# APRIL-ZJU/Ctrl-VIO

Measured on AMD Instinct MI355X. Metric: sliding-window solves/sec (10 KF, 200 lm, 2000 IMU), higher is better.
Workload: dtype f64; 1 GPU; config2: 10 KF / 200 landmarks / 2000 IMU sliding window (K = 24 knots, 814 reprojection blocks), <= 15 LM iterations (Ceres 1.14 trust region + projected line search); distinct_windows_per_gpu=64, streams_per_gpu=4, concurrent_solves_per_gpu=2

## Files before the change

ctrl-vio_amd/csrc/kernels.hpp:

```cpp
#pragma once
#include <utility>

#include "device_types.hpp"
#include "factors.hpp"

namespace ctv {

enum { LIN_AT_X = 0,
       LIN_SPEC = 1,
       COST_AT_X = 2 };
__device__ __forceinline__ bool lin_run(const Lm &lm, int mode) { return lm.status == 0 && (mode != LIN_SPEC || lm.step_valid != 0); }
__device__ __forceinline__ bool lin_cost_only(const Lm &lm, int mode, const LmParams &p) {
  return mode == COST_AT_X || (mode == LIN_SPEC && lm.iter >= p.max_iters && lm.ls_active == 0);
}
__device__ __forceinline__ int lin_target(const Lm &lm, int mode) { return mode == LIN_SPEC ? 1 - lm.cur : lm.cur; }

__device__ __forceinline__ double grad_norm_entry(const Dev &d, const WinMeta &m, int w, int j, const double *g, bool at_cand);
__device__ __forceinline__ void begin_iteration(const Dev &d, int w, int *s_go);

__device__ __forceinline__ double readlane_d(double x, int lane) {
  const long long b = __double_as_longlong(x);
  const int lo = __builtin_amdgcn_readlane((int)(b & 0xffffffffll), lane);
  const int hi = __builtin_amdgcn_readlane((int)(b >> 32), lane);
  return __longlong_as_double(((long long)hi << 32) | (unsigned int)lo);
}

__device__ __forceinline__ int opaque_zero() {
  int z;
  asm volatile("s_mov_b32 %0, 0" : "=s"(z));
  return z;
}

__device__ __forceinline__ void lds_wave_sync() {
  __builtin_amdgcn_s_waitcnt(0xc07f);
  __builtin_amdgcn_wave_barrier();
}
__device__ __forceinline__ void lds_block_sync() {
  __builtin_amdgcn_s_waitcnt(0xc07f);
  __builtin_amdgcn_s_barrier();
}

#define CTV_STAMP(stamps, idx, cap, lane_cond, ...)                                                        \
  do {                                                                                                     \
    if ((stamps) && (lane_cond) && (idx) < (cap))                                                          \
      (stamps)[(idx)++] = clock64() __VA_OPT__(+ (long long)((__VA_ARGS__) * 0.0));                        \
  } while (0)

__device__ __forceinline__ int imu_col(int c, int s, int K, int bias) {
  if (c < 12) return 6 * (s + c / 3) + c % 3;
  if (c < 24) return 6 * (s + (c - 12) / 3) + 3 + (c - 12) % 3;
  return 6 * K + 6 * bias + (c - 24);
}
__device__ __forceinline__ int vis_col(int c, int si, int sj, int P) {
  if (c < 12) return 6 * (si + c / 3) + c % 3;
  if (c < 24) return 6 * (si + (c - 12) / 3) + 3 + (c - 12) % 3;
  if (c < 36) return 6 * (sj + (c - 24) / 3) + (c - 24) % 3;
  if (c < 48) return 6 * (sj + (c - 36) / 3) + 3 + (c - 36) % 3;
  if (c == 48) return -1;
  return P - 1;
}

__device__ __forceinline__ void load_knots(const double *quat, const double *pos, int k0, const double *origin,
                                                            Knots4 &k) {
#pragma unroll
  for (int i = 0; i < 4; ++i) {
    const double *q = quat + 4 * (k0 + i), *p = pos + 3 * (k0 + i);
    k.q[i] = qmk(q[0], q[1], q[2], q[3]);
    k.p[i] = mk(p[0] - origin[0], p[1] - origin[1], p[2] - origin[2]);
  }
}

struct LocalFrame {
  Q4 qref_inv;
  M3 RT;
  double o[3];
  __device__ __forceinline__ void init(const double *quat, const double *pos, int kref) {
    const double *q = quat + 4 * kref, *p = pos + 3 * kref;
    qref_inv = qmk(-q[0], -q[1], -q[2], q[3]);
    const M3 R = q2R(qmk(q[0], q[1], q[2], q[3]));
#pragma unroll
    for (int i = 0; i < 3; ++i)
#pragma unroll
      for (int j = 0; j < 3; ++j) RT.m[3 * i + j] = R.m[3 * j + i];
    o[0] = p[0]; o[1] = p[1]; o[2] = p[2];
  }
  __device__ __forceinline__ void load(const double *quat, const double *pos, int k0, Knots4 &k) const {
#pragma unroll
    for (int i = 0; i < 4; ++i) {
      const double *q = quat + 4 * (k0 + i), *p = pos + 3 * (k0 + i);
      k.q[i] = qmul_raw(qref_inv, qmk(q[0], q[1], q[2], q[3]));
      k.p[i] = mul(RT, mk(p[0] - o[0], p[1] - o[1], p[2] - o[2]));
    }
  }
  __device__ __forceinline__ V3 rotate(const double *v) const { return mul(RT, mk(v[0], v[1], v[2])); }
  __device__ __forceinline__ M3 RrefT() const { return RT; }
};

}

#include "kernels_control.hpp"
#include "kernels_imu.hpp"
#include "kernels_visual.hpp"
#include "kernels_assemble.hpp"
#include "kernels_solve.hpp"
#include "kernels_query.hpp"
#include "kernels_cov.hpp"
#include "kernels_tri.hpp"
```

ctrl-vio_amd/csrc/kernels_assemble.hpp:

```cpp
#pragma once

namespace ctv {

__device__ __forceinline__ double prior_H(const Dev &d, const WinMeta &m, int ga, int gb) {
  if (m.pn <= 0) return 0.0;
  const int pi = d.pinv[m.p0 + ga], pj = d.pinv[m.p0 + gb];
  return (pi >= 0 && pj >= 0) ? d.pH[m.pH0 + (size_t)pi * m.pn + pj] : 0.0;
}
__device__ __forceinline__ double prior_g(const Dev &d, const WinMeta &m, int u) {
  if (m.pn <= 0) return 0.0;
  const int pi = d.pinv[m.p0 + u];
  return pi >= 0 ? d.pgrad[m.pv0 + pi] : 0.0;
}
__device__ __forceinline__ void packed_decode(int i, int tri, int K6, int P, int &ga, int &gb) {
  if (i < tri) {
    ga = (int)((sqrtf(8.0f * (float)i + 1.0f) - 1.0f) * 0.5f);
    ga += ((ga + 1) * (ga + 2) / 2 <= i) ? 1 : 0;
    ga -= (ga * (ga + 1) / 2 > i) ? 1 : 0;
    gb = i - ga * (ga + 1) / 2;
  } else {
    ga = P - 1;
    gb = (i - tri) < K6 ? (i - tri) : P - 1;
  }
}
__device__ __forceinline__ void bias_rows_store(const Dev &d, const WinMeta &m, int tg, const double *bias, int first, int stride) {
  const int K = m.K, F = m.F, P = m.P, K6 = 6 * K, ldh = m.ldh, nbr = 6 * F;
  double *Hg = d.HppS[tg] + m.H0, *g = d.gS[tg] + m.u0;
  const int32_t *boff = d.bgl_off + m.bias0 + (int)(&m - d.wins);
  const int n_rect = nbr * K6, n_tri = nbr * (nbr + 1) / 2, n_ld = nbr, n_g = nbr;
  for (int e = first; e < n_rect + n_tri + n_ld + n_g; e += stride) {
    if (e < n_rect + n_tri) {
      int rb, c;
      if (e < n_rect) { rb = e / K6; c = e - rb * K6; }
      else {
        const int t = e - n_rect;
        int i2 = (int)((sqrtf(8.0f * (float)t + 1.0f) - 1.0f) * 0.5f);
        i2 += ((i2 + 1) * (i2 + 2) / 2 <= t) ? 1 : 0;
        i2 -= (i2 * (i2 + 1) / 2 > t) ? 1 : 0;
        rb = i2; c = K6 + t - i2 * (i2 + 1) / 2;
      }
      const int f = rb / 6, a = rb - 6 * f, r = K6 + rb;
      double v = 0.0;
      const int g0 = boff[f], g1 = boff[f + 1];
      if (c < K6) {
        const int k = c / 6, cc = c - 6 * k;
        for (int q = g0; q < g1; ++q) {
          const int gi = d.bgl[q];
          const int sg = d.groups[gi].s;
          if (k >= sg && k <= sg + 3) v += d.imu_tiles[(size_t)gi * 1024 + (24 + a) * 32 + (cc < 3 ? 3 * (k - sg) + cc : 12 + 3 * (k - sg) + cc - 3)];
        }
      } else {
        const int cb = c - K6, f2 = cb / 6, a2 = cb - 6 * f2;
        if (f2 == f)
          for (int q = g0; q < g1; ++q) v += d.imu_tiles[(size_t)d.bgl[q] * 1024 + (24 + a) * 32 + 24 + a2];
        if (a2 == a)
          for (int b = 0; b < m.NB; ++b) {
            const int bi = d.bc_i[m.bc0 + b], bj = d.bc_j[m.bc0 + b];
            const double wv = d.bc_w[(size_t)(m.bc0 + b) * 6 + a];
            if (f2 == f) { if (bi == f) v += wv * wv; if (bj == f) v += wv * wv; }
            else if ((bi == f2 && bj == f) || (bi == f && bj == f2)) v -= wv * wv;
          }
      }
      Hg[(long long)r * ldh + c] = v + prior_H(d, m, r, c);
    } else if (e < n_rect + n_tri + n_ld) {
      const int c = K6 + e - n_rect - n_tri;
      Hg[(long long)(P - 1) * ldh + c] = prior_H(d, m, P - 1, c);
    } else {
      const int rb = e - n_rect - n_tri - n_ld, f = rb / 6, a = rb - 6 * f, r = K6 + rb;
      double v = 0.0;
      for (int q = boff[f]; q < boff[f + 1]; ++q) v += d.imu_tiles[(size_t)d.bgl[q] * 1024 + (24 + a) * 32 + 30];
      for (int b = 0; b < m.NB; ++b) {
        const int bi = d.bc_i[m.bc0 + b], bj = d.bc_j[m.bc0 + b];
        if (bi != f && bj != f) continue;
        const double wv = d.bc_w[(size_t)(m.bc0 + b) * 6 + a];
        const double rr = wv * (bias[6 * (m.bias0 + bj) + a] - bias[6 * (m.bias0 + bi) + a]);
        if (bi == f) v -= wv * rr;
        if (bj == f) v += wv * rr;
      }
      g[r] = v + prior_g(d, m, r);
    }
  }
}

constexpr int VIS_SROWS = 116;
constexpr int vis_stage_stride(int ch) { return ch + 1; }
constexpr size_t vis_stage_bytes(int nw, int ch) { return (size_t)nw * VIS_SROWS * vis_stage_stride(ch) * sizeof(double) + (size_t)nw * 2 * ch * sizeof(int); }
__device__ __forceinline__ f64x4 mfma16(double a, double b, f64x4 c) { return __builtin_amdgcn_mfma_f64_16x16x4f64(a, b, c, 0, 0, 0); }
template <int CH, bool LDSH, int NW = 8, bool STORE = false> __global__ __launch_bounds__(64 * NW) void k_assemble_vis_mfma(Dev d, int mode) {
  typedef f64x4 acc_t;
  constexpr int CHP = vis_stage_stride(CH), RPP = 64 / CH, NT = 64 * NW;
  static_assert(!STORE || LDSH, "the store-semantics tail needs the LDS-resident Hessian");
  static_assert(CH == 8, "the staging pattern is written for items of 8 blocks");
  constexpr int SROWS = VIS_SROWS, NEXP = 48 / RPP;
  const long long t_begin = d.dbg ? clock64() : 0;
  const int w = blockIdx.x, part = blockIdx.y, nparts = gridDim.y;
  if (!lin_run(d.lm[w], mode) || lin_cost_only(d.lm[w], mode, d.prm)) return;
  const WinMeta &m = d.wins[w];
  const int tgset = lin_target(d.lm[w], mode);
  const int P = m.P, K = m.K, nvitem = m.nvitem, vitem0 = m.vitem0, ngrp = m.ngrp, grp0 = m.grp0, u0 = m.u0, ldh = m.ldh;
  if ((m.vis_lds != 0) != LDSH) return;
  if (!LDSH && m.V == 0) return;
  extern __shared__ __attribute__((aligned(16))) unsigned char smv[];
  double *Hs = reinterpret_cast<double *>(smv);
  const int K6 = 6 * K, tri = K6 * (K6 + 1) / 2;
  const int nHh = LDSH ? tri + K6 + 1 : 0;
  const int nH = nHh + K6 + 1;
  double *gs = Hs + nHh;
  double *stage = reinterpret_cast<double *>(Hs + ((nH + 3) & ~3));
  int *keys = reinterpret_cast<int *>(stage + NW * SROWS * CHP);
  const int tid = threadIdx.x, wave = tid >> 6, lane = tid & 63;
  const int per_round = NW * nparts;
  constexpr int NGI = 3;
  double tv[NGI][9], tgv[NGI];
  int gs_[NGI], gb_[NGI];
  if (LDSH) {
#pragma unroll
    for (int u = 0; u < NGI; ++u) {
      const int gi = min(part * NW + wave + u * per_round, max(ngrp - 1, 0));
      const ImuGroup grp = d.groups[grp0 + gi];
      gs_[u] = grp.s; gb_[u] = grp.bias;
      const double *tile = d.imu_tiles + (size_t)(grp0 + gi) * 1024;
#pragma unroll
      for (int q = 0; q < 9; ++q) { const int e = lane + 64 * q; tv[u][q] = ngrp > 0 ? tile[(e / 24) * 32 + e % 24] : 0.0; }
      tgv[u] = (STORE && ngrp > 0) ? tile[min(lane, 23) * 32 + 30] : 0.0;
    }
  }
  for (int i = 2 * tid; i < ((nH + 3) & ~3); i += 2 * NT) *reinterpret_cast<double2 *>(Hs + i) = double2{0.0, 0.0};
  __syncthreads();
  if (LDSH) {
#pragma unroll
    for (int u = 0; u < NGI; ++u) {
      if (part * NW + wave + u * per_round >= ngrp) continue;
#pragma unroll
      for (int q = 0; q < 9; ++q) {
        const int e = lane + 64 * q, a = e / 24, b = e % 24;
        const int ga = imu_col(a, gs_[u], K, gb_[u]), gb = imu_col(b, gs_[u], K, gb_[u]);
        if (ga >= gb) atomicAdd(&Hs[ga * (ga + 1) / 2 + gb], tv[u][q]);
      }
      if (STORE && lane < 24) atomicAdd(&Hs[nHh + imu_col(lane, gs_[u], K, gb_[u])], tgv[u]);
    }
  }
  double *Js = stage + wave * SROWS * CHP;
  int *ks = keys + wave * 2 * CH;
  const size_t V = (size_t)d.Vtot;
  const int it0 = (int)((long long)nvitem * (part * NW + wave) / per_round);
  const int rounds = (int)((long long)nvitem * (part * NW + wave + 1) / per_round) - it0;
  double *Hg = d.HppS[tgset] + m.H0;
  const int q4 = lane >> 4, l15 = lane & 15, bsel = q4 >> 1, rr = q4 & 1;
  const int sc = lane % CH, srr = lane / CH;
  long long *dbg = (d.dbg && w == (d.nwin > 1000 ? 1000 : 0) && part == 0) ? d.dbg + 48 : nullptr;
  int dbi = 0;
  if (dbg && tid == 0) dbg[dbi++] = t_begin;
  CTV_STAMP(dbg, dbi, 15, tid == 0);
  int orow[3];
#pragma unroll
  for (int I = 0; I < 3; ++I) orow[I] = (2 * (16 * I + l15) + rr) * CHP;
  const int ldrow = (98 + rr) * CHP, rrow = (100 + rr) * CHP;
  double tj[5], tg9[9], tc0 = 0.0;
  int n = 0, v0 = 0, key_i = 0, key_j = 0;
  int my_start, my_count;
  {
    const int it = it0 + lane;
    const VisItem I = d.vitems[vitem0 + min(it, max(nvitem - 1, 0))];
    my_start = I.start;
    my_count = (lane < rounds && it < nvitem) ? I.count : 0;
  }
  auto item_desc = [&](int r, int &istart, int &icount) {
    if (r < 64) { istart = __shfl(my_start, r); icount = __shfl(my_count, r); }
    else {
      const int it = it0 + r;
      const VisItem I = d.vitems[vitem0 + min(it, nvitem - 1)];
      istart = I.start; icount = (r < rounds && it < nvitem) ? I.count : 0;
    }
    if (r >= rounds) icount = 0;
  };
  int idn = 0, idkn = 0, ian = 0, iakn = 0;
  auto load_ids = [&](int r) {
    int istart, icount;
    item_desc(r, istart, icount);
    idn = d.vblk[istart + (sc < icount ? sc : 0)];
    ian = d.vblk_anc[istart + (sc < icount ? sc : 0)];
    idkn = d.vblk[istart + (lane < icount ? lane : 0)];
    iakn = d.vblk_anc[istart + (lane < icount ? lane : 0)];
  };
  auto fetch = [&](int r) {
    int istart, icount;
    item_desc(r, istart, icount);
    n = icount;
    v0 = istart;
    const unsigned jb = (unsigned)idn * (unsigned)VT_ROWS + (unsigned)srr;
#pragma unroll
    for (int i = 0; i < 3; ++i) tj[i] = d.Jt[jb + (unsigned)(8 * i)];
    tj[3] = d.Jt[jb + 26u];
    tj[4] = d.Jt[(unsigned)idn * (unsigned)VT_ROWS + (unsigned)min(34 + srr, VT_ROWS - 1)];
    const double *rec = d.arec + (size_t)ian * AREC;
#pragma unroll
    for (int i = 0; i < 3; ++i)
#pragma unroll
      for (int mm = 0; mm < 3; ++mm) tg9[3 * i + mm] = rec[AR_GR + 3 * ((srr + 8 * i) >> 1) + mm];
    tc0 = rec[AR_CP0 + (srr & 3)];
    key_i = d.a_s[iakn];
    key_j = d.vsj[idkn];
    load_ids(r + 1);
  };
  if (nvitem > 0) load_ids(0);
  if (nvitem > 0) fetch(0);
  acc_t acc[6];
  double pl[3], pr[3], pll, prl;
  int asi = -1, asj = -1;
  auto reset_acc = [&]() {
#pragma unroll
    for (int q = 0; q < 6; ++q) acc[q] = acc_t{0.0, 0.0, 0.0, 0.0};
#pragma unroll
    for (int I = 0; I < 3; ++I) { pl[I] = 0.0; pr[I] = 0.0; }
    pll = 0.0; prl = 0.0;
  };
  auto scatter = [&](int si, int sj) {
#pragma unroll
    for (int I = 0; I < 3; ++I) {
      pl[I] += __shfl_xor(pl[I], 16); pl[I] += __shfl_xor(pl[I], 32);
      pr[I] += __shfl_xor(pr[I], 16); pr[I] += __shfl_xor(pr[I], 32);
    }
    pll += __shfl_xor(pll, 16); pll += __shfl_xor(pll, 32);
    prl += __shfl_xor(prl, 16); prl += __shfl_xor(prl, 32);
    int gcol[3], tcol[3], grow[3][4], trow[3][4];
#pragma unroll
    for (int J = 0; J < 3; ++J) {
      gcol[J] = vis_col(16 * J + l15, si, sj, P);
      tcol[J] = gcol[J] * (gcol[J] + 1) / 2;
#pragma unroll
      for (int rg = 0; rg < 4; ++rg) {
        grow[J][rg] = vis_col(16 * J + (q4 + 4 * rg), si, sj, P);
        trow[J][rg] = grow[J][rg] * (grow[J][rg] + 1) / 2;
      }
    }
    int q = 0;
#pragma unroll
    for (int I = 0; I < 3; ++I)
#pragma unroll
      for (int J = 0; J <= I; ++J, ++q) {
#pragma unroll
        for (int rg = 0; rg < 4; ++rg) {
          const int ca = 16 * I + (q4 + 4 * rg), cb = 16 * J + l15;
          if (I == J && ca < cb) continue;
          const int gA = grow[I][rg], gB = gcol[J];
          double hv = acc[q][rg];
          if (gA == gB && ca != cb) hv *= 2.0;
          const bool ge = gA >= gB;
          if (LDSH) atomicAdd(&Hs[(ge ? trow[I][rg] : tcol[J]) + (ge ? gB : gA)], hv);
          else atomicAdd(&Hg[(long long)(ge ? gA : gB) * ldh + (ge ? gB : gA)], hv);
        }
      }
    if (q4 == 0) {
#pragma unroll
      for (int J = 0; J < 3; ++J) {
        if (LDSH) atomicAdd(&Hs[tri + gcol[J]], pl[J]);
        else atomicAdd(&Hg[(long long)(P - 1) * ldh + gcol[J]], pl[J]);
        atomicAdd(&gs[gcol[J]], pr[J]);
      }
      if (l15 == 0) {
        if (LDSH) atomicAdd(&Hs[tri + K6], pll);
        else atomicAdd(&Hg[(long long)(P - 1) * ldh + (P - 1)], pll);
        atomicAdd(&gs[K6], prl);
      }
    }
  };
  for (int r = 0; r < rounds && nvitem > 0; ++r) {
    const int ncur = n;
    {
      const bool in = sc < ncur;
#pragma unroll
      for (int i = 0; i < 3; ++i) Js[(48 + srr + 8 * i) * CHP + sc] = in ? tj[i] : 0.0;
      Js[(98 + srr) * CHP + sc] = in ? tj[3] : 0.0;
      if (srr < 2) Js[(106 + srr) * CHP + sc] = in ? tj[4] : 0.0;
      else if (srr < 6) Js[(110 + srr) * CHP + sc] = in ? tj[4] : 0.0;
      if (srr < 4) Js[(108 + srr) * CHP + sc] = in ? tc0 : 0.0;
    }
    if (lane < CH) { ks[lane] = key_i; ks[CH + lane] = key_j; }
    __builtin_amdgcn_wave_barrier();
    {
      const int rr2 = srr & 1;
      const double a0 = Js[(102 + rr2) * CHP + sc], a1 = Js[(104 + rr2) * CHP + sc], a2 = Js[(106 + rr2) * CHP + sc];
#pragma unroll
      for (int i = 0; i < 3; ++i) Js[(srr + 8 * i) * CHP + sc] = a0 * tg9[3 * i] + a1 * tg9[3 * i + 1] + a2 * tg9[3 * i + 2];
    }
#pragma unroll
    for (int e = 0; e < NEXP; ++e) {
      constexpr int HALF = 24 / RPP;
      const int side = e / HALF, rem = (e % HALF) * RPP + srr;
      const int pc = rem >> 1, kk = pc / 3, b = pc - 3 * kk;
      const double pv = Js[(102 + 2 * b + (rem & 1)) * CHP + sc], cv = Js[(108 + 4 * side + kk) * CHP + sc];
      Js[(24 + 48 * side + rem) * CHP + sc] = side ? -(cv * pv) : cv * pv;
    }
    __builtin_amdgcn_wave_barrier();
    if (r < 2) CTV_STAMP(dbg, dbi, 15, tid == 0);
    fetch(r + 1);
    int start = 0;
    while (start < ncur) {
      const int si = ks[start], sj = ks[CH + start];
      const bool diff = (lane > start && lane < ncur) && (ks[lane] != si || ks[CH + lane] != sj);
      const unsigned long long mask = __ballot(diff);
      const int end = mask ? (__ffsll((long long)mask) - 1) : ncur;
      if (asi != si || asj != sj) {
        if (asi >= 0) scatter(asi, asj);
        reset_acc();
        asi = si; asj = sj;
      }
      for (int v8 = start; v8 < end; v8 += 8) {
        double a[4][3], ldv[4], rv[4];
        const bool nomask = end == ncur && v8 + 8 <= CH;
#pragma unroll
        for (int s = 0; s < 4; ++s) {
          const int blk = v8 + 2 * s + bsel;
          const int bc = min(blk, CH);
#pragma unroll
          for (int I = 0; I < 3; ++I) a[s][I] = Js[orow[I] + bc];
          ldv[s] = Js[ldrow + bc];
          rv[s] = Js[rrow + bc];
        }
        if (!nomask) {
#pragma unroll
          for (int s = 0; s < 4; ++s) {
            const bool in = v8 + 2 * s + bsel < end;
#pragma unroll
            for (int I = 0; I < 3; ++I) a[s][I] = in ? a[s][I] : 0.0;
            ldv[s] = in ? ldv[s] : 0.0;
            rv[s] = in ? rv[s] : 0.0;
          }
        }
#pragma unroll
        for (int s = 0; s < 4; ++s) {
          if (v8 + 2 * s >= end) break;
          int q = 0;
#pragma unroll
          for (int I = 0; I < 3; ++I)
#pragma unroll
            for (int J = 0; J <= I; ++J, ++q) acc[q] = mfma16(a[s][I], a[s][J], acc[q]);
#pragma unroll
          for (int I = 0; I < 3; ++I) { pl[I] += a[s][I] * ldv[s]; pr[I] += a[s][I] * rv[s]; }
          pll += ldv[s] * ldv[s];
          prl += rv[s] * ldv[s];
        }
      }
      if (r < 2) CTV_STAMP(dbg, dbi, 15, tid == 0);
      start = end;
    }
    if (r < 2) CTV_STAMP(dbg, dbi, 15, tid == 0);
  }
  if (asi >= 0) scatter(asi, asj);
  __syncthreads();
  CTV_STAMP(dbg, dbi, 15, tid == 0);
  for (int gi = part * NW + wave + NGI * per_round; LDSH && gi < ngrp; gi += per_round) {
    const ImuGroup grp = d.groups[grp0 + gi];
    const double *tile = d.imu_tiles + (size_t)(grp0 + gi) * 1024;
    double tv[9];
#pragma unroll
    for (int u = 0; u < 9; ++u) { const int e = lane + 64 * u; tv[u] = tile[(e / 24) * 32 + e % 24]; }
#pragma unroll
    for (int u = 0; u < 9; ++u) {
      const int e = lane + 64 * u, a = e / 24, b = e % 24;
      const int ga = imu_col(a, grp.s, K, grp.bias), gb = imu_col(b, grp.s, K, grp.bias);
      if (ga >= gb) atomicAdd(&Hs[ga * (ga + 1) / 2 + gb], tv[u]);
    }
    if (STORE && lane < 24) atomicAdd(&gs[imu_col(lane, grp.s, K, grp.bias)], tile[lane * 32 + 30]);
  }
  __syncthreads();
  CTV_STAMP(dbg, dbi, 15, tid == 0);
  if constexpr (STORE) {
    if (nparts > 1) {
      double *dst = d.Hpart + ((size_t)w * nparts + part) * d.npart_stride;
      for (int i = tid; i < nH; i += NT) dst[i] = Hs[i];
      return;
    }
    double *gq = d.gS[tgset] + u0;
    for (int i0 = tid; i0 < nHh; i0 += 4 * NT) {
      double hv4[4];
#pragma unroll
      for (int u = 0; u < 4; ++u) hv4[u] = Hs[min(i0 + NT * u, nHh - 1)];
#pragma unroll
      for (int u = 0; u < 4; ++u) {
        const int i = i0 + NT * u;
        if (i >= nHh) continue;
        int ga, gb;
        packed_decode(i, tri, K6, P, ga, gb);
        Hg[(long long)ga * ldh + gb] = hv4[u] + prior_H(d, m, ga, gb);
      }
    }
    for (int i = tid; i < K6 + 1; i += NT) { const int uu = i < K6 ? i : P - 1; gq[uu] = gs[i] + prior_g(d, m, uu); }
    return;
  }
  for (int i0 = tid; LDSH && i0 < nHh; i0 += 4 * NT) {
    double hv4[4];
#pragma unroll
    for (int u = 0; u < 4; ++u) hv4[u] = Hs[min(i0 + NT * u, nHh - 1)];
#pragma unroll
    for (int u = 0; u < 4; ++u) {
      const int i = i0 + NT * u;
      const double hv = hv4[u];
      if (i >= nHh || (nparts > 1 && hv == 0.0)) continue;
      int ga, gb;
      packed_decode(i, tri, K6, P, ga, gb);
      if (nparts > 1) atomicAdd(&Hg[(long long)ga * ldh + gb], hv);
      else Hg[(long long)ga * ldh + gb] = hv;
    }
  }
  CTV_STAMP(dbg, dbi, 15, tid == 0);
  for (int i = tid; i < K6 + 1; i += NT) {
    const double gv = gs[i];
    if (gv != 0.0) atomicAdd(&d.gS[tgset][u0 + (i < K6 ? i : P - 1)], gv);
  }
  CTV_STAMP(dbg, dbi, 15, tid == 0);
}

__global__ __launch_bounds__(256) void k_bias_rows(Dev d, int mode) {
  const int w = blockIdx.y;
  if (!lin_run(d.lm[w], mode) || lin_cost_only(d.lm[w], mode, d.prm)) return;
  const WinMeta &m = d.wins[w];
  if (!m.vis_lds) return;
  bias_rows_store(d, m, lin_target(d.lm[w], mode), mode == LIN_SPEC ? d.cbias : d.bias, blockIdx.x * blockDim.x + threadIdx.x, gridDim.x * blockDim.x);
}

__global__ __launch_bounds__(256) void k_reduce_finalize(Dev d, int mode, int nparts) {
  const int w = blockIdx.y;
  if (!lin_run(d.lm[w], mode) || lin_cost_only(d.lm[w], mode, d.prm)) return;
  const WinMeta &m = d.wins[w];
  if (!m.vis_lds) return;
  const int tg = lin_target(d.lm[w], mode);
  const int P = m.P, K6 = 6 * m.K, tri = K6 * (K6 + 1) / 2, nHh = tri + K6 + 1, nH = nHh + K6 + 1, ldh = m.ldh;
  double *Hg = d.HppS[tg] + m.H0, *g = d.gS[tg] + m.u0;
  const double *src = d.Hpart + (size_t)w * nparts * d.npart_stride;
  const int first = blockIdx.x * blockDim.x + threadIdx.x, stride = gridDim.x * blockDim.x;
  for (int i = first; i < nH; i += stride) {
    double v = 0.0;
    int p = 0;
    for (; p + 8 <= nparts; p += 8) {
      double t8[8];
#pragma unroll
      for (int q = 0; q < 8; ++q) t8[q] = src[(size_t)(p + q) * d.npart_stride + i];
#pragma unroll
      for (int q = 0; q < 8; ++q) v += t8[q];
    }
    for (; p < nparts; ++p) v += src[(size_t)p * d.npart_stride + i];
    if (i < nHh) {
      int ga, gb;
      packed_decode(i, tri, K6, P, ga, gb);
      Hg[(long long)ga * ldh + gb] = v + prior_H(d, m, ga, gb);
    } else {
      const int uu = (i - nHh) < K6 ? (i - nHh) : P - 1;
      g[uu] = v + prior_g(d, m, uu);
    }
  }
  bias_rows_store(d, m, tg, mode == LIN_SPEC ? d.cbias : d.bias, first, stride);
}

constexpr int VX_COLS = 50, VX_LD = 2 * VX_COLS + 2;
__global__ __launch_bounds__(256) void k_vis_expand(Dev d, int mode) {
  const long long e = (long long)blockIdx.x * blockDim.x + threadIdx.x;
  if (e >= (long long)d.Vtot * (VX_COLS + 1)) return;
  const int pos = (int)(e / (VX_COLS + 1)), c = (int)(e - (long long)pos * (VX_COLS + 1));
  const int w = d.vb_win[pos / 64];
  const WinMeta &m = d.wins[w];
  if (pos - m.vis0 >= m.V) return;
  if (!lin_run(d.lm[w], mode) || lin_cost_only(d.lm[w], mode, d.prm) || m.vis_lds) return;
  const int slot = m.vis0 + d.vrow[pos];
  double *out = d.vexp + (size_t)pos * VX_LD;
  if (c == VX_COLS) { out[2 * VX_COLS] = (double)d.a_s[d.v_anc[slot]]; out[2 * VX_COLS + 1] = (double)d.vsj[slot]; return; }
  const double *J = d.Jt + (size_t)slot * VT_ROWS;
#pragma unroll
  for (int rr = 0; rr < 2; ++rr) {
    double v;
    if (c < 12) {
      const double *gr = d.arec + (size_t)d.v_anc[slot] * AREC + AR_GR + 3 * c;
      v = J[VB_AT + rr] * gr[0] + J[VB_AT + 2 + rr] * gr[1] + J[VB_AT + 4 + rr] * gr[2];
    } else if (c < 24) {
      const int k = (c - 12) / 3, b = (c - 12) % 3;
      v = d.arec[(size_t)d.v_anc[slot] * AREC + AR_CP0 + k] * J[VB_AT + 2 * b + rr];
    } else if (c < 36) {
      v = J[VB_JROT + 2 * (c - 24) + rr];
    } else if (c < 48) {
      const int k = (c - 36) / 3, b = (c - 36) % 3;
      v = -(J[VB_CP1 + k] * J[VB_AT + 2 * b + rr]);
    } else {
      v = J[(c == 48 ? VB_LD : VB_RES) + rr];
    }
    out[VX_COLS * rr + c] = v;
  }
}
// ... 295 lines not shown
```

ctrl-vio_amd/csrc/kernels_solve.hpp:

```cpp
#pragma once

namespace ctv {

__device__ __forceinline__ void begin_iteration(const Dev &d, int w, int *s_go) {
  Lm &lm = d.lm[w];
  if (threadIdx.x == 0) {
    int go = 0;
    if (!lm.status) {
      if (lm.ls_active) atomicAdd(d.n_active, 1);
      else if (lm.iter >= d.prm.max_iters) lm.status = 1 + 0;
      else if (lm.last_ok && __longlong_as_double((long long)lm.gmax_bits) <= d.prm.gtol) lm.status = 1 + 1;
      else if (lm.mu <= d.prm.min_radius) lm.status = 1 + 4;
      else {
        lm.iter += 1;
        lm.accept = 0; lm.step_valid = 0; lm.chol_fail = 0; lm.alpha = 1.0;
        atomicAdd(d.n_active, 1);
        go = 1;
      }
    }
    *s_go = go;
  }
  __syncthreads();
  if (!*s_go) return;
  const WinMeta &m = d.wins[w];
// ... 686 lines not shown
      const int j = min(j0, max(jb - 1, 0)), ja = max(j, ca), jc = max(j, cb);
#pragma unroll
      for (int ii = 0; ii < 32; ++ii) lv[ii] = S[(long long)(jb + min(ii, nb - 1)) * ldh + (ii < 16 ? ja : jc)];
    }
    if (wave == 0) {
      const double *gi = d.chol_inv + ((size_t)w * d.chol_nblk + b) * 1024;
      double li[32];
      const int l31 = lane & 31;
#pragma unroll
      for (int i = 0; i < 32; ++i) li[i] = gi[i * 32 + l31];
      double acc = 0.0;
#pragma unroll
      for (int i = 0; i < 32; ++i) acc += li[i] * ((i < nb) ? xs[jb + i] : 0.0);
      __builtin_amdgcn_wave_barrier();
      if (lane < nb) { xs[jb + lane] = acc; yb[lane] = acc; }
    }
    __syncthreads();
    if (upd) {
      double sacc = 0.0;
      const bool ma = j0 >= ca, mb = j0 >= cb;
#pragma unroll
      for (int ii = 0; ii < 32; ++ii) sacc += ((ii < 16 ? ma : mb) && ii < nb) ? lv[ii] * yb[ii] : 0.0;
      xs[j0] -= sacc;
    }
    for (int j = j0 + NT; j < jb; j += NT) {
      double sacc = 0.0;
      for (int ii = 0; ii < nb; ++ii) sacc += (j >= (ii < 16 ? ca : cb)) ? S[(long long)(jb + ii) * ldh + j] * yb[ii] : 0.0;
      xs[j] -= sacc;
    }
    __syncthreads();
  }
  for (int i = tid; i < P; i += NT) x[i] = xs[i];
  CTV_STAMP(dbg, dbi, 30, tid == 0);
  if (tid == 0) lm.chol_fail = s_fail;
}

template <int C> __device__ __forceinline__ void chol_dpp_update(double &vc, double m, double vj) {
  asm("s_nop 1\n\tv_fmac_f64_dpp %0, -%1, %2 row_newbcast:%3 row_mask:0xf bank_mask:0xf" : "+v"(vc) : "v"(m), "v"(vj), "n"(C));
}
template <int C> __device__ __forceinline__ void chol_dpp_update4(double &v0, double &v1, double &v2, double &v3, double m, double vj) {
  asm("s_nop 1\n\tv_fmac_f64_dpp %0, -%4, %5 row_newbcast:%6 row_mask:0xf bank_mask:0xf\n\t"
      "v_fmac_f64_dpp %1, -%4, %5 row_newbcast:%7 row_mask:0xf bank_mask:0xf\n\t"
      "v_fmac_f64_dpp %2, -%4, %5 row_newbcast:%8 row_mask:0xf bank_mask:0xf\n\t"
      "v_fmac_f64_dpp %3, -%4, %5 row_newbcast:%9 row_mask:0xf bank_mask:0xf"
      : "+v"(v0), "+v"(v1), "+v"(v2), "+v"(v3)
      : "v"(m), "v"(vj), "n"(C), "n"(C + 1), "n"(C + 2), "n"(C + 3));
}
template <int J, int C> __device__ __forceinline__ void chol16_dpp_rest(double (&v)[16], double m) {
  if constexpr (C + 3 <= 15) {
    chol_dpp_update4<C>(v[C], v[C + 1], v[C + 2], v[C + 3], m, v[J]);
    chol16_dpp_rest<J, C + 4>(v, m);
  } else if constexpr (C <= 15) {
    chol_dpp_update<C>(v[C], m, v[J]);
    chol16_dpp_rest<J, C + 1>(v, m);
  }
}
__device__ __forceinline__ double chol_pivot_rsqrt3(double p) {
  const double y = __builtin_amdgcn_rsq(p);
  const double e = __builtin_fma(-(p * y), y, 1.0);
  return __builtin_fma(y * e, __builtin_fma(0.375, e, 0.5), y);
}
template <int J, bool FULL> __device__ __forceinline__ void chol16_dpp_from(double (&v)[16], double d, int nreal) {
  v[J] *= d;
  if constexpr (J < 15) {
    const unsigned lo = (unsigned)__double2loint(v[J]), hi = (unsigned)__double2hiint(v[J]);
    const auto slo = __builtin_amdgcn_permlane16_swap(lo, lo, false, false);
    const auto shi = __builtin_amdgcn_permlane16_swap(hi, hi, false, false);
    const double m = __hiloint2double((int)shi[0], (int)slo[0]);
    chol_dpp_update<J + 1>(v[J + 1], m, v[J]);
    double dn = chol_pivot_rsqrt3(readlane_d(v[J + 1], J + 1));
    if constexpr (!FULL) dn = (J + 1 < nreal) ? dn : 1.0;
    if constexpr (J < 14) chol16_dpp_rest<J, J + 2>(v, m);
    chol16_dpp_from<J + 1, FULL>(v, dn, nreal);
  }
}
__device__ __forceinline__ void chol16_dpp(double (&v)[16], int nreal, int &bad) {
  const double d0 = chol_pivot_rsqrt3(readlane_d(v[0], 0));
  if (nreal >= 16) chol16_dpp_from<0, true>(v, d0, nreal);
  else chol16_dpp_from<0, false>(v, nreal > 0 ? d0 : 1.0, nreal);
  const double last = readlane_d(v[15], 15);
  if (!(last - last == 0.0)) bad = 1;
}

__device__ __forceinline__ double rowgroup_sum(double p) {
  unsigned lo = (unsigned)__double2loint(p), hi = (unsigned)__double2hiint(p);
  const auto a = __builtin_amdgcn_permlane16_swap(lo, lo, false, false);
  const auto b = __builtin_amdgcn_permlane16_swap(hi, hi, false, false);
  const double s = __hiloint2double((int)b[0], (int)a[0]) + __hiloint2double((int)b[1], (int)a[1]);
  lo = (unsigned)__double2loint(s); hi = (unsigned)__double2hiint(s);
  const auto c = __builtin_amdgcn_permlane32_swap(lo, lo, false, false);
  const auto e = __builtin_amdgcn_permlane32_swap(hi, hi, false, false);
  return __hiloint2double((int)e[0], (int)c[0]) + __hiloint2double((int)e[1], (int)c[1]);
}
template <int K> __device__ __forceinline__ void dpp_dot16(double &acc, double t, const double (&lk)[16]) {
  if constexpr (K < 16) {
    asm("s_nop 1\n\tv_fmac_f64_dpp %0, %1, %2 row_newbcast:%3 row_mask:0xf bank_mask:0xf" : "+v"(acc) : "v"(t), "v"(lk[K]), "n"(K));
    dpp_dot16<K + 1>(acc, t, lk);
  }
}
__device__ __forceinline__ double f64x4_get(const f64x4 &a, int r) { return r == 0 ? a[0] : (r == 1 ? a[1] : (r == 2 ? a[2] : a[3])); }

constexpr int CHOL_NS = 7;

struct CholActive {
  unsigned long long w[4];
  __device__ __forceinline__ int bit(int i) const {
    const unsigned long long wlo = (i & 128) ? w[2] : w[0], whi = (i & 128) ? w[3] : w[1];
    return (int)((((i & 64) ? whi : wlo) >> (i & 63)) & 1ull);
  }
};
struct CholWindow {
  const double *S, *Hc, *y, *dd;
  int P, ldh, K6;
  bool from_h;
  CholActive act;
  __device__ __forceinline__ bool plain(int a, int b) const {
    const SchurTiles tiles{K6, P};
    return from_h && !(tiles.nz_row(a) && tiles.nz_col(b));
  }
};
__device__ __forceinline__ CholWindow chol_window(const Dev &d, const WinMeta &m, const Lm &lm, int lane) {
  CholWindow cw = {d.S + m.H0, d.HppS[lm.cur] + m.H0, d.rhs + m.p0, d.dd + m.u0, m.P, m.ldh, 6 * m.K, d.schur_plain_in_H != 0, {{0ull, 0ull, 0ull, 0ull}}};
  if (cw.from_h) {
    unsigned char ab[4];
#pragma unroll
    for (int k = 0; k < 4; ++k) ab[k] = d.active[m.u0 + min(lane + 64 * k, cw.P - 1)];
#pragma unroll
    for (int k = 0; k < 4; ++k) cw.act.w[k] = __ballot(lane + 64 * k < cw.P && ab[k] != 0);
  }
  return cw;
}
__device__ __forceinline__ int chol_first_panel(const Dev &d, const WinMeta &m, int a, int b) {
  return __builtin_amdgcn_readfirstlane(max(d.env_tile[m.tr0 + a], d.env_tile[m.tr0 + b]));
}
__device__ __forceinline__ void chol_tile_fetch(f64x4 &t, const CholWindow &cw, int a, int b, int q4, int l15) {
  const double *S = cw.S, *Hc = cw.Hc;
  const double *src = cw.plain(a, b) ? Hc : S;
#pragma unroll
  for (int r = 0; r < 4; ++r) {
    const int rc = min(16 * a + q4 + 4 * r, cw.P - 1);
    t[r] = src[(long long)rc * cw.ldh + min(16 * b + l15, rc)];
  }
}
__device__ __forceinline__ void chol_tile_fixup(f64x4 &t, const CholWindow &cw, int a, int b, int q4, int l15) {
  const int P = cw.P, ip = P / 16, col = 16 * b + l15;
  if (cw.plain(a, b)) {
    const int a_j = cw.act.bit(col);
    double ddiag = 0.0;
    if (a == b) ddiag = cw.dd[min(col, P - 1)];
#pragma unroll
    for (int r = 0; r < 4; ++r) {
      const int row = 16 * a + q4 + 4 * r;
      t[r] = (cw.act.bit(row) & a_j) ? t[r] + (row == col ? ddiag : 0.0) : (row == col ? 1.0 : 0.0);
    }
  }
  if (a == b) {
#pragma unroll
    for (int r = 0; r < 4; ++r) t[r] = (col <= 16 * a + q4 + 4 * r) ? t[r] : 0.0;
  }
  if (a == ip) {
    const double yv = cw.y[min(col, P - 1)];
#pragma unroll
    for (int r = 0; r < 4; ++r) {
      const int row = 16 * ip + q4 + 4 * r;
      t[r] = row < P ? t[r] : (row == P ? (col < P ? yv : 0.0) : (row == col ? 1.0 : 0.0));
    }
  }
}
__device__ __forceinline__ void chol_tile_to_lds(double *blk, const f64x4 &t, int q4, int l15) {
#pragma unroll
  for (int r = 0; r < 4; ++r) blk[(q4 + 4 * r) * 17 + l15] = t[r];
}
__device__ __forceinline__ int chol_diag_tile(double *Dg, const double *Id, int k, int P, int ip, int rp, double *tv, int lane) {
  const int l15 = lane & 15;
  double v[16];
  const int opaque0 = opaque_zero();
// ... 549 lines not shown
```

Baseline: 47560 solves/s.

## Reorder visual Jacobian rows knot-major and simplify Hessian scatter indexing

Stages the visual Jacobian columns in knot-major order so that global Hessian row and column indices become affine in the knot offsets. This lets the scatter skip per-element vis_col decoding and the diagonal-doubling checks when the two spans don't overlap (sj-si>=4). IMU tile scatter now uses precomputed per-lane packed offsets with a wave-uniform span, and cross-lane reductions use permlane swaps instead of shuffles. The LDS-to-global flush now walks rows directly instead of inverting the packed triangular index with a sqrt. These changes add code size and register pressure, and they depend on the permutation being correct, which a static_assert checks.

```diff
diff --git a/ctrl-vio_amd/csrc/kernels.hpp b/ctrl-vio_amd/csrc/kernels.hpp
--- a/ctrl-vio_amd/csrc/kernels.hpp
+++ b/ctrl-vio_amd/csrc/kernels.hpp
@@ -23,6 +23,17 @@
   const int lo = __builtin_amdgcn_readlane((int)(b & 0xffffffffll), lane);
   const int hi = __builtin_amdgcn_readlane((int)(b >> 32), lane);
   return __longlong_as_double(((long long)hi << 32) | (unsigned int)lo);
+}
+
+__device__ __forceinline__ double rowgroup_sum(double p) {
+  unsigned lo = (unsigned)__double2loint(p), hi = (unsigned)__double2hiint(p);
+  const auto a = __builtin_amdgcn_permlane16_swap(lo, lo, false, false);
+  const auto b = __builtin_amdgcn_permlane16_swap(hi, hi, false, false);
+  const double s = __hiloint2double((int)b[0], (int)a[0]) + __hiloint2double((int)b[1], (int)a[1]);
+  lo = (unsigned)__double2loint(s); hi = (unsigned)__double2hiint(s);
+  const auto c = __builtin_amdgcn_permlane32_swap(lo, lo, false, false);
+  const auto e = __builtin_amdgcn_permlane32_swap(hi, hi, false, false);
+  return __hiloint2double((int)e[0], (int)c[0]) + __hiloint2double((int)e[1], (int)c[1]);
 }
 
 __device__ __forceinline__ int opaque_zero() {
@@ -51,7 +62,7 @@
   if (c < 24) return 6 * (s + (c - 12) / 3) + 3 + (c - 12) % 3;
   return 6 * K + 6 * bias + (c - 24);
 }
-__device__ __forceinline__ int vis_col(int c, int si, int sj, int P) {
+constexpr __device__ __forceinline__ int vis_col(int c, int si, int sj, int P) {
   if (c < 12) return 6 * (si + c / 3) + c % 3;
   if (c < 24) return 6 * (si + (c - 12) / 3) + 3 + (c - 12) % 3;
   if (c < 36) return 6 * (sj + (c - 24) / 3) + (c - 24) % 3;
@@ -59,6 +70,23 @@
   if (c == 48) return -1;
   return P - 1;
 }
+constexpr __device__ __forceinline__ int vis_knot_major_to_col(int c) {
+  const int end = c / 24, r = c % 24, k = r / 6, cc = r % 6;
+  return 24 * end + (cc < 3 ? 3 * k + cc : 12 + 3 * k + (cc - 3));
+}
+constexpr bool vis_knot_major_complete() {
+  bool seen[48] = {};
+  for (int c = 0; c < 48; ++c) {
+    const int o = vis_knot_major_to_col(c);
+    if (o < 0 || o >= 48 || seen[o]) return false;
+    seen[o] = true;
+    for (int si = 0; si < 3; ++si)
+      for (int sj = 0; sj < 9; sj += 4)
+        if (vis_col(o, si, sj, 1000) != (c < 24 ? 6 * si + c : 6 * sj + c - 24)) return false;
+  }
+  return true;
+}
+static_assert(vis_knot_major_complete(), "vis_knot_major_to_col must permute the 48 pose columns into [end][knot][6]");
 
 __device__ __forceinline__ void load_knots(const double *quat, const double *pos, int k0, const double *origin,
                                                             Knots4 &k) {
diff --git a/ctrl-vio_amd/csrc/kernels_assemble.hpp b/ctrl-vio_amd/csrc/kernels_assemble.hpp
--- a/ctrl-vio_amd/csrc/kernels_assemble.hpp
+++ b/ctrl-vio_amd/csrc/kernels_assemble.hpp
@@ -86,6 +86,16 @@
 constexpr int vis_stage_stride(int ch) { return ch + 1; }
 constexpr size_t vis_stage_bytes(int nw, int ch) { return (size_t)nw * VIS_SROWS * vis_stage_stride(ch) * sizeof(double) + (size_t)nw * 2 * ch * sizeof(int); }
 __device__ __forceinline__ f64x4 mfma16(double a, double b, f64x4 c) { return __builtin_amdgcn_mfma_f64_16x16x4f64(a, b, c, 0, 0, 0); }
+__device__ __forceinline__ int imu_tile_const(int e) {
+  const int oa = imu_col(e / 24, 0, 0, 0), ob = imu_col(e % 24, 0, 0, 0);
+  return oa >= ob ? ((oa + 1) << 16) | (oa * (oa + 1) / 2 + ob) : -1;
+}
+__device__ __forceinline__ void imu_tile_add(double *Hs, int s, const int (&tc)[9], const double (&tv)[9]) {
+  const int B = 6 * s, tB = B * (B + 1) / 2;
+#pragma unroll
+  for (int q = 0; q < 9; ++q)
+    if (tc[q] >= 0) atomicAdd(&Hs[tB + (int)__umul24((unsigned)B, (unsigned)tc[q] >> 16) + (tc[q] & 0xffff)], tv[q]);
+}
 template <int CH, bool LDSH, int NW = 8, bool STORE = false> __global__ __launch_bounds__(64 * NW) void k_assemble_vis_mfma(Dev d, int mode) {
   typedef f64x4 acc_t;
   constexpr int CHP = vis_stage_stride(CH), RPP = 64 / CH, NT = 64 * NW;
@@ -108,17 +118,17 @@
   double *gs = Hs + nHh;
   double *stage = reinterpret_cast<double *>(Hs + ((nH + 3) & ~3));
   int *keys = reinterpret_cast<int *>(stage + NW * SROWS * CHP);
-  const int tid = threadIdx.x, wave = tid >> 6, lane = tid & 63;
+  const int tid = threadIdx.x, wave = __builtin_amdgcn_readfirstlane(tid >> 6), lane = tid & 63;
   const int per_round = NW * nparts;
   constexpr int NGI = 3;
   double tv[NGI][9], tgv[NGI];
-  int gs_[NGI], gb_[NGI];
+  int gs_[NGI];
   if (LDSH) {
 #pragma unroll
     for (int u = 0; u < NGI; ++u) {
       const int gi = min(part * NW + wave + u * per_round, max(ngrp - 1, 0));
       const ImuGroup grp = d.groups[grp0 + gi];
-      gs_[u] = grp.s; gb_[u] = grp.bias;
+      gs_[u] = grp.s;
       const double *tile = d.imu_tiles + (size_t)(grp0 + gi) * 1024;
 #pragma unroll
       for (int q = 0; q < 9; ++q) { const int e = lane + 64 * q; tv[u][q] = ngrp > 0 ? tile[(e / 24) * 32 + e % 24] : 0.0; }
@@ -128,16 +138,16 @@
   for (int i = 2 * tid; i < ((nH + 3) & ~3); i += 2 * NT) *reinterpret_cast<double2 *>(Hs + i) = double2{0.0, 0.0};
   __syncthreads();
   if (LDSH) {
+    int tc[9];
+#pragma unroll
+    for (int q = 0; q < 9; ++q) tc[q] = imu_tile_const(lane + 64 * q);
+    const int tcg = imu_col(min(lane, 23), 0, 0, 0);
 #pragma unroll
     for (int u = 0; u < NGI; ++u) {
       if (part * NW + wave + u * per_round >= ngrp) continue;
-#pragma unroll
-      for (int q = 0; q < 9; ++q) {
-        const int e = lane + 64 * q, a = e / 24, b = e % 24;
-        const int ga = imu_col(a, gs_[u], K, gb_[u]), gb = imu_col(b, gs_[u], K, gb_[u]);
-        if (ga >= gb) atomicAdd(&Hs[ga * (ga + 1) / 2 + gb], tv[u][q]);
-      }
-      if (STORE && lane < 24) atomicAdd(&Hs[nHh + imu_col(lane, gs_[u], K, gb_[u])], tgv[u]);
+      const int sg = __builtin_amdgcn_readfirstlane(gs_[u]);
+      imu_tile_add(Hs, sg, tc, tv[u]);
+      if (STORE && lane < 24) atomicAdd(&Hs[nHh + 6 * sg + tcg], tgv[u]);
     }
   }
   double *Js = stage + wave * SROWS * CHP;
@@ -154,7 +164,7 @@
   CTV_STAMP(dbg, dbi, 15, tid == 0);
   int orow[3];
 #pragma unroll
-  for (int I = 0; I < 3; ++I) orow[I] = (2 * (16 * I + l15) + rr) * CHP;
+  for (int I = 0; I < 3; ++I) orow[I] = (2 * vis_knot_major_to_col(16 * I + l15) + rr) * CHP;
   const int ldrow = (98 + rr) * CHP, rrow = (100 + rr) * CHP;
   double tj[5], tg9[9], tc0 = 0.0;
   int n = 0, v0 = 0, key_i = 0, key_j = 0;
@@ -166,7 +176,7 @@
     my_count = (lane < rounds && it < nvitem) ? I.count : 0;
   }
   auto item_desc = [&](int r, int &istart, int &icount) {
-    if (r < 64) { istart = __shfl(my_start, r); icount = __shfl(my_count, r); }
+    if (r < 64) { istart = __builtin_amdgcn_readlane(my_start, r); icount = __builtin_amdgcn_readlane(my_count, r); }
     else {
       const int it = it0 + r;
       const VisItem I = d.vitems[vitem0 + min(it, nvitem - 1)];
@@ -217,40 +227,54 @@
   };
   auto scatter = [&](int si, int sj) {
 #pragma unroll
+    for (int I = 0; I < 3; ++I) { pl[I] = rowgroup_sum(pl[I]); pr[I] = rowgroup_sum(pr[I]); }
+    pll = rowgroup_sum(pll); prl = rowgroup_sum(prl);
+    const int bi = 6 * si, bj = 6 * sj - 24;
+    int gcol[3], grow[3][4], trow[3][4];
+    gcol[0] = bi + l15; gcol[1] = 16 + l15 + (l15 < 8 ? bi : bj); gcol[2] = bj + 32 + l15;
+#pragma unroll
     for (int I = 0; I < 3; ++I) {
-      pl[I] += __shfl_xor(pl[I], 16); pl[I] += __shfl_xor(pl[I], 32);
-      pr[I] += __shfl_xor(pr[I], 16); pr[I] += __shfl_xor(pr[I], 32);
-    }
-    pll += __shfl_xor(pll, 16); pll += __shfl_xor(pll, 32);
-    prl += __shfl_xor(prl, 16); prl += __shfl_xor(prl, 32);
-    int gcol[3], tcol[3], grow[3][4], trow[3][4];
-#pragma unroll
-    for (int J = 0; J < 3; ++J) {
-      gcol[J] = vis_col(16 * J + l15, si, sj, P);
-      tcol[J] = gcol[J] * (gcol[J] + 1) / 2;
-#pragma unroll
-      for (int rg = 0; rg < 4; ++rg) {
-        grow[J][rg] = vis_col(16 * J + (q4 + 4 * rg), si, sj, P);
-        trow[J][rg] = grow[J][rg] * (grow[J][rg] + 1) / 2;
-      }
-    }
-    int q = 0;
-#pragma unroll
-    for (int I = 0; I < 3; ++I)
-#pragma unroll
-      for (int J = 0; J <= I; ++J, ++q) {
-#pragma unroll
-        for (int rg = 0; rg < 4; ++rg) {
-          const int ca = 16 * I + (q4 + 4 * rg), cb = 16 * J + l15;
-          if (I == J && ca < cb) continue;
-          const int gA = grow[I][rg], gB = gcol[J];
-          double hv = acc[q][rg];
-          if (gA == gB && ca != cb) hv *= 2.0;
-          const bool ge = gA >= gB;
-          if (LDSH) atomicAdd(&Hs[(ge ? trow[I][rg] : tcol[J]) + (ge ? gB : gA)], hv);
-          else atomicAdd(&Hg[(long long)(ge ? gA : gB) * ldh + (ge ? gB : gA)], hv);
+      const int g0 = 16 * I + q4 + (I == 0 ? bi : bj), g1 = 16 * I + q4 + (I == 2 ? bj : bi);
+      grow[I][0] = g1; grow[I][1] = g1 + 4; grow[I][2] = g0 + 8; grow[I][3] = g0 + 12;
+      trow[I][0] = g1 * (g1 + 1) / 2; trow[I][1] = trow[I][0] + 4 * g1 + 10;
+      trow[I][2] = I == 1 ? (g0 + 8) * (g0 + 9) / 2 : trow[I][1] + 4 * g1 + 26;
+      trow[I][3] = trow[I][2] + 4 * g0 + 42;
+    }
+    if (sj - si >= 4) {
+      int q = 0;
+#pragma unroll
+      for (int I = 0; I < 3; ++I)
+#pragma unroll
+        for (int J = 0; J <= I; ++J, ++q) {
+#pragma unroll
+          for (int rg = 0; rg < 4; ++rg) {
+            if (I == J && q4 + 4 * rg < l15) continue;
+            if (LDSH) atomicAdd(&Hs[trow[I][rg] + gcol[J]], acc[q][rg]);
+            else atomicAdd(&Hg[(long long)grow[I][rg] * ldh + gcol[J]], acc[q][rg]);
+          }
         }
-      }
+    } else {
+      int tcol[3];
+#pragma unroll
+      for (int J = 0; J < 3; ++J) tcol[J] = gcol[J] * (gcol[J] + 1) / 2;
+      int q = 0;
+#pragma unroll
+      for (int I = 0; I < 3; ++I)
+#pragma unroll
+        for (int J = 0; J <= I; ++J, ++q) {
+#pragma unroll
+          for (int rg = 0; rg < 4; ++rg) {
+            const int ca = 16 * I + (q4 + 4 * rg), cb = 16 * J + l15;
+            if (I == J && ca < cb) continue;
+            const int gA = grow[I][rg], gB = gcol[J];
+            double hv = acc[q][rg];
+            if (gA == gB && ca != cb) hv *= 2.0;
+            const bool ge = gA >= gB;
+            if (LDSH) atomicAdd(&Hs[(ge ? trow[I][rg] : tcol[J]) + (ge ? gB : gA)], hv);
+            else atomicAdd(&Hg[(long long)(ge ? gA : gB) * ldh + (ge ? gB : gA)], hv);
+          }
+        }
+    }
     if (q4 == 0) {
 #pragma unroll
       for (int J = 0; J < 3; ++J) {
@@ -281,16 +305,22 @@
     {
       const int rr2 = srr & 1;
       const double a0 = Js[(102 + rr2) * CHP + sc], a1 = Js[(104 + rr2) * CHP + sc], a2 = Js[(106 + rr2) * CHP + sc];
+      constexpr int HALF = 24 / RPP;
+      double pv[HALF], cv[2][HALF];
+#pragma unroll
+      for (int h = 0; h < HALF; ++h) {
+        const int rem = h * RPP + srr, pc = rem >> 1, kk = pc / 3, b = pc - 3 * kk;
+        pv[h] = Js[(102 + 2 * b + (rem & 1)) * CHP + sc];
+        cv[0][h] = Js[(108 + kk) * CHP + sc];
+        cv[1][h] = Js[(112 + kk) * CHP + sc];
+      }
 #pragma unroll
       for (int i = 0; i < 3; ++i) Js[(srr + 8 * i) * CHP + sc] = a0 * tg9[3 * i] + a1 * tg9[3 * i + 1] + a2 * tg9[3 * i + 2];
-    }
-#pragma unroll
-    for (int e = 0; e < NEXP; ++e) {
-      constexpr int HALF = 24 / RPP;
-      const int side = e / HALF, rem = (e % HALF) * RPP + srr;
-      const int pc = rem >> 1, kk = pc / 3, b = pc - 3 * kk;
-      const double pv = Js[(102 + 2 * b + (rem & 1)) * CHP + sc], cv = Js[(108 + 4 * side + kk) * CHP + sc];
-      Js[(24 + 48 * side + rem) * CHP + sc] = side ? -(cv * pv) : cv * pv;
+#pragma unroll
+      for (int e = 0; e < NEXP; ++e) {
+        const int side = e / HALF, h = e % HALF;
+        Js[(24 + 48 * side + h * RPP + srr) * CHP + sc] = side ? -(cv[1][h] * pv[h]) : cv[0][h] * pv[h];
+      }
     }
     __builtin_amdgcn_wave_barrier();
     if (r < 2) CTV_STAMP(dbg, dbi, 15, tid == 0);
@@ -350,19 +380,21 @@
   if (asi >= 0) scatter(asi, asj);
   __syncthreads();
   CTV_STAMP(dbg, dbi, 15, tid == 0);
-  for (int gi = part * NW + wave + NGI * per_round; LDSH && gi < ngrp; gi += per_round) {
-    const ImuGroup grp = d.groups[grp0 + gi];
-    const double *tile = d.imu_tiles + (size_t)(grp0 + gi) * 1024;
-    double tv[9];
-#pragma unroll
-    for (int u = 0; u < 9; ++u) { const int e = lane + 64 * u; tv[u] = tile[(e / 24) * 32 + e % 24]; }
-#pragma unroll
-    for (int u = 0; u < 9; ++u) {
-      const int e = lane + 64 * u, a = e / 24, b = e % 24;
-      const int ga = imu_col(a, grp.s, K, grp.bias), gb = imu_col(b, grp.s, K, grp.bias);
-      if (ga >= gb) atomicAdd(&Hs[ga * (ga + 1) / 2 + gb], tv[u]);
-    }
-    if (STORE && lane < 24) atomicAdd(&gs[imu_col(lane, grp.s, K, grp.bias)], tile[lane * 32 + 30]);
+  if (LDSH && part * NW + wave + NGI * per_round < ngrp) {
+    const int ln = lane + opaque_zero();
+    int tc[9];
+#pragma unroll
+    for (int q = 0; q < 9; ++q) tc[q] = imu_tile_const(ln + 64 * q);
+    const int tcg = imu_col(min(ln, 23), 0, 0, 0);
+    for (int gi = part * NW + wave + NGI * per_round; gi < ngrp; gi += per_round) {
+      const int s = __builtin_amdgcn_readfirstlane(d.groups[grp0 + gi].s);
+      const double *tile = d.imu_tiles + (size_t)(grp0 + gi) * 1024;
+      double tv[9];
+#pragma unroll
+      for (int u = 0; u < 9; ++u) { const int e = lane + 64 * u; tv[u] = tile[(e / 24) * 32 + e % 24]; }
+      imu_tile_add(Hs, s, tc, tv);
+      if (STORE && lane < 24) atomicAdd(&gs[6 * s + tcg], tile[lane * 32 + 30]);
+    }
   }
   __syncthreads();
   CTV_STAMP(dbg, dbi, 15, tid == 0);
@@ -373,36 +405,20 @@
       return;
     }
     double *gq = d.gS[tgset] + u0;
-    for (int i0 = tid; i0 < nHh; i0 += 4 * NT) {
-      double hv4[4];
-#pragma unroll
-      for (int u = 0; u < 4; ++u) hv4[u] = Hs[min(i0 + NT * u, nHh - 1)];
-#pragma unroll
-      for (int u = 0; u < 4; ++u) {
-        const int i = i0 + NT * u;
-        if (i >= nHh) continue;
-        int ga, gb;
-        packed_decode(i, tri, K6, P, ga, gb);
-        Hg[(long long)ga * ldh + gb] = hv4[u] + prior_H(d, m, ga, gb);
-      }
-    }
+    for (int ga = wave; ga < K6; ga += NW)
+      for (int gb = lane; gb <= ga; gb += 64) Hg[(long long)ga * ldh + gb] = Hs[ga * (ga + 1) / 2 + gb] + prior_H(d, m, ga, gb);
+    for (int i = tid; i < K6 + 1; i += NT) { const int gb = i < K6 ? i : P - 1; Hg[(long long)(P - 1) * ldh + gb] = Hs[tri + i] + prior_H(d, m, P - 1, gb); }
     for (int i = tid; i < K6 + 1; i += NT) { const int uu = i < K6 ? i : P - 1; gq[uu] = gs[i] + prior_g(d, m, uu); }
     return;
   }
-  for (int i0 = tid; LDSH && i0 < nHh; i0 += 4 * NT) {
-    double hv4[4];
-#pragma unroll
-    for (int u = 0; u < 4; ++u) hv4[u] = Hs[min(i0 + NT * u, nHh - 1)];
-#pragma unroll
-    for (int u = 0; u < 4; ++u) {
-      const int i = i0 + NT * u;
-      const double hv = hv4[u];
-      if (i >= nHh || (nparts > 1 && hv == 0.0)) continue;
-      int ga, gb;
-      packed_decode(i, tri, K6, P, ga, gb);
-      if (nparts > 1) atomicAdd(&Hg[(long long)ga * ldh + gb], hv);
+  if (LDSH) {
+    auto flush = [&](int ga, int gb, double hv) {
+      if (nparts > 1) { if (hv != 0.0) atomicAdd(&Hg[(long long)ga * ldh + gb], hv); }
       else Hg[(long long)ga * ldh + gb] = hv;
-    }
+    };
+    for (int ga = wave; ga < K6; ga += NW)
+      for (int gb = lane; gb <= ga; gb += 64) flush(ga, gb, Hs[ga * (ga + 1) / 2 + gb]);
+    for (int i = tid; i < K6 + 1; i += NT) flush(P - 1, i < K6 ? i : P - 1, Hs[tri + i]);
   }
   CTV_STAMP(dbg, dbi, 15, tid == 0);
   for (int i = tid; i < K6 + 1; i += NT) {
diff --git a/ctrl-vio_amd/csrc/kernels_solve.hpp b/ctrl-vio_amd/csrc/kernels_solve.hpp
--- a/ctrl-vio_amd/csrc/kernels_solve.hpp
+++ b/ctrl-vio_amd/csrc/kernels_solve.hpp
@@ -792,16 +792,6 @@
   if (!(last - last == 0.0)) bad = 1;
 }
 
-__device__ __forceinline__ double rowgroup_sum(double p) {
-  unsigned lo = (unsigned)__double2loint(p), hi = (unsigned)__double2hiint(p);
-  const auto a = __builtin_amdgcn_permlane16_swap(lo, lo, false, false);
-  const auto b = __builtin_amdgcn_permlane16_swap(hi, hi, false, false);
-  const double s = __hiloint2double((int)b[0], (int)a[0]) + __hiloint2double((int)b[1], (int)a[1]);
-  lo = (unsigned)__double2loint(s); hi = (unsigned)__double2hiint(s);
-  const auto c = __builtin_amdgcn_permlane32_swap(lo, lo, false, false);
-  const auto e = __builtin_amdgcn_permlane32_swap(hi, hi, false, false);
-  return __hiloint2double((int)e[0], (int)c[0]) + __hiloint2double((int)e[1], (int)c[1]);
-}
 template <int K> __device__ __forceinline__ void dpp_dot16(double &acc, double t, const double (&lk)[16]) {
   if constexpr (K < 16) {
     asm("s_nop 1\n\tv_fmac_f64_dpp %0, %1, %2 row_newbcast:%3 row_mask:0xf bank_mask:0xf" : "+v"(acc) : "v"(t), "v"(lk[K]), "n"(K));
```

Result: faster. 48740 solves/s (median of 6 runs) (+2.5%).
